# Toytiny/CMFlow

Hardware: AMD Instinct MI355X
Metric: frame-pairs/sec CMFlow fwd+bwd (higher is better)
Workload: dtype f32; 1 GPU; cmflow fwd+bwd training (7 cross-modal losses + Adam, train-mode BN) step, N=256, B=64 per GPU (global 64), ball-query r=2/4/8/16 K=4/8/16/32, kNN K=8; synthetic clouds, seeded random-init weights; parallelism=dp1

## Files before the change

### cmflow_amd/_lib.py

```python
import ctypes
import os
import subprocess

import torch

_HERE = os.path.dirname(os.path.abspath(__file__))
SO_PATH = os.environ.get("CMF_LIB") or os.path.join(_HERE, "libcmflow_hip.so")

_vp, _ci, _cf, _ll = ctypes.c_void_p, ctypes.c_int, ctypes.c_float, ctypes.c_longlong

SIGNATURES = {
    "cmf_ball_query": [_ci, _ci, _ci, _cf, _ci, _vp, _vp, _vp, _vp],
    "cmf_ball_query_multi": [_ci, _ci, _ci, _ci, _vp, _vp, _ci, _vp, _vp, _vp, _ci, _vp],
    "cmf_setconv_queries": [_ci, _vp, _vp],
    "cmf_ball_query_multi_counted": [_ci, _ci, _ci, _ci, _vp, _vp, _ci, _vp, _vp, _vp, _vp, _vp, _vp],
    "cmf_setconv_queries_counted": [_ci, _vp, _vp, _vp],
    "cmf_knn_counted": [_ci, _ci, _ci, _ci, _vp, _vp, _vp, _vp, _vp, _vp],
    "cmf_global_max_cat_counted": [_ci, _ci, _ci, _vp, _ll, _vp, _ll, _vp, _vp, _vp],
    "cmf_ego_refine_counted": [_ci, _ci, _cf, _cf, _vp, _vp, _vp, _vp, _vp, _vp, _vp, _vp, _vp, _vp, _vp, _vp],
    "cmf_eval_metrics_counted": [_ci, _ci, _vp, _vp, _vp, _vp, _vp, _vp, _vp, _vp, _cf, _cf, _cf, _vp, _vp, _vp],
    "cmf_ego_refine_grad_counted": [_ci, _ci, _cf, _vp, _vp, _vp, _vp, _vp, _vp, _vp, _vp, _vp, _vp, _vp, _vp, _vp],
    "cmf_global_max_cat_grad_counted": [_ci, _ci, _ci, _vp, _ll, _vp, _vp, _ll, _vp, _vp],
    "cmf_radar_loss_counted_workspace": [_ci, _ci, _ci, _ci],
    "cmf_radar_loss_counted_workspace_tiled": [_ci, _ci, _ci, _ci],
# ... 49 lines not shown
    "cmf_three_nn": [_ci, _ci, _ci, _vp, _vp, _vp, _vp, _vp],
    "cmf_three_interpolate": [_ci, _ci, _ci, _ci, _vp, _vp, _vp, _vp, _vp],
    "cmf_three_interpolate_grad": [_ci, _ci, _ci, _ci, _vp, _vp, _vp, _vp, _vp],
    "cmf_bn_finalize": [_ci, _ci, ctypes.c_double, _vp, _vp, _vp, _cf, _cf, _vp, _vp, _vp, _vp, _vp, _vp, _vp, _vp],
    "cmf_colsum_finalize": [_ci, _ci, _vp, _vp, _vp, _vp, _vp],
    "cmf_group_affine": [_ci, _ci, _ci, _ci, _ci, _vp, _ci, _vp, _ci, _vp, _vp, _vp, _ci, _vp, _ci, _vp, _vp, _vp, _vp, _vp],
    "cmf_adam_step": [_ci, _vp, _vp, _ll, _vp, _vp, _vp, ctypes.c_double, ctypes.c_double, ctypes.c_double, ctypes.c_double, ctypes.c_double, _ll, _vp],
    "cmf_group_prep": [_ci, _ci, _ci, _ci, _ci, _vp, _vp, _vp, _ci, _vp, _vp, _vp, _vp, _vp],
    "cmf_gemm_gather_affine": [_ci, _ci, _ci, _vp, _ll, _vp, _vp, _vp, _vp, _vp, _vp, _ll, _vp, _ll, _vp, _vp],
    "cmf_gemm_dx_gather": [_ci, _ci, _ci, _vp, _ll, _vp, _ll, _vp, _ll, _vp, _ll, _vp, _vp, _vp, _vp, _vp, _vp, _vp, _vp, _vp],
    "cmf_group_perm": [_ci, _ci, _vp, _vp, _vp, _vp, _vp, _vp, _vp],
    "cmf_gemm_dx_gather_sum": [_ci, _ci, _ci, _vp, _ll, _vp, _ll, _vp, _ll, _vp, _vp, _vp, _vp, _vp, _vp, _vp, _vp, _vp, _vp, _vp],
    "cmf_group_rows_grad_bn_cf_pieces": [_ci, _ci, _ci, _ci, _ci, _vp, _vp, _ll, _vp, _ll, _vp, _vp, _vp, _vp, _vp, _vp, _cf, _vp, _vp, _vp,
                                         _ci, _vp],
    "cmf_gemm_dw_gather_split": [_ci, _ci, _ll],
    "cmf_gemm_dw_gather_bn_bwd": [_ci, _ci, _ll, _vp, _ll, _vp, _ll, _vp, _vp, _vp, _vp, _vp, _ll, _vp, _ll, _vp, _vp, _vp, _vp, _vp, _vp, _ll,
                                  _ci, _vp, _ci, _vp],
    "cmf_gemm_dw_gather": [_ci, _ci, _ll, _vp, _ll, _vp, _ll, _vp, _vp, _vp, _vp, _vp, _vp, _ll, _ci, _vp, _ci, _vp],
    "cmf_colsum": [_ci, _ci, _vp, _vp, _ci, _vp, _vp, _vp],
    "cmf_setconv_dwx": [_ci, _cf, _ci, _vp, _vp, _vp, _vp, _vp, _vp, _ci, _ci, _vp],
    "cmf_group_rows_grad_bn": [_ci, _ci, _ci, _ci, _vp, _vp, _vp, _vp, _vp, _vp, _cf, _vp, _vp, _vp, _ci, _vp],
    "cmf_group_rows_grad_bn_cf": [_ci, _ci, _ci, _ci, _ci, _vp, _vp, _ll, _vp, _ll, _vp, _vp, _vp, _vp, _vp, _vp, _cf, _vp, _vp, _vp,
                                  _ci, _vp],
    "cmf_bn_relu_maxpool": [_ll, _ci, _ci, _vp, _vp, _vp, _vp, _ll, _vp, _vp],
    "cmf_maxpool_bwd": [_ll, _ci, _ci, _vp, _ll, _vp, _vp, _vp, _vp, _vp, _vp, _vp, _vp, _vp],
    "cmf_affine_relu": [_ll, _ci, _vp, _ll, _vp, _vp, _vp, _ll, _vp],
    "cmf_act_bwd_stats": [_ll, _ci, _vp, _ll, _vp, _ll, _vp, _vp, _vp, _vp, _vp, _vp, _vp],
    "cmf_bn_bwd_apply": [_ll, _ci, _vp, _vp, _ll, _vp, _vp, _vp, _vp, _vp],
    "cmf_maxpool_bwd_point": [_ll, _ci, _ci, _vp, _ll, _vp, _vp, _vp, _vp, _vp, _vp, _vp, _vp, _vp],
    "cmf_thin_bwd_layer_pooled": [_ll, _ci, _ci, _ci, _vp, _vp, _vp, _vp, _vp, _vp, _vp, _vp, _vp, _vp, _vp, _vp, _vp, _vp, _vp, _vp,
                                  _ci, _vp, _vp],
    "cmf_thin_bwd_wide_supported": [_ci, _ci],
    "cmf_thin_bwd_wide_slabs": [_ll, _ci, _vp],
    "cmf_thin_bwd_wide_layer": [_ll, _ci, _vp, _ll, _vp, _vp, _ci, _vp, _ll, _vp, _vp, _vp, _vp, _vp, _ll, _vp, _ll,
                                _vp, _vp, _vp, _vp, _vp, _ll, _vp, _vp, _ll, _ci, _vp, _vp],
    "cmf_thin_bwd_supported": [_ci, _ci],
    "cmf_thin_bwd_slabs": [_ll, _vp],
    "cmf_thin_bwd_layer": [_ll, _ci, _ci, _vp, _ll, _vp, _ll, _vp, _vp, _vp, _vp, _vp, _ll, _vp, _ll, _ci,
                           _vp, _vp, _vp, _vp, _vp, _vp, _ll, _vp, _vp, _ll, _ci, _vp, _vp],
    "cmf_weighted_ksum": [_ll, _ci, _ci, _ci, _ci, _vp, _vp, _vp, _vp, _vp],
    "cmf_weighted_ksum_grad_tiles": [_ci],
    "cmf_weighted_ksum_grad": [_ll, _ci, _ci, _ci, _ci, _ci, _vp, _vp, _vp, _vp, _vp, _vp, _vp, _vp],
    "cmf_weightnet_ksum_tiles": [_ci],
    "cmf_weightnet_ksum": [_ll, _ci, _ci, _ci, _ci, _vp, _vp, _vp, _vp, _vp, _vp, _vp],
    "cmf_weightnet_ksum_grad": [_ll, _ci, _ci, _ci, _ci, _ci, _vp, _ll, _vp, _vp, _vp, _vp, _vp, _vp, _vp, _vp, _vp],
    "cmf_global_max_cat": [_ci, _ci, _ci, _vp, _ll, _vp, _ll, _vp, _vp],
# ... 168 lines not shown
```

### cmflow_amd/csrc/cmf_common.h

```cpp
#pragma once
#include <hip/hip_runtime.h>
#include <atomic>
#include <mutex>
#include <stdint.h>
#include <stdlib.h>

#define CMF_WAVE 64

#define CMF_CHECK_ARG(cond) \
    do { if (!(cond)) return (int)hipErrorInvalidValue; } while (0)

static inline int cmf_launch_status() { return (int)hipGetLastError(); }

static inline int cmf_divup(long long a, long long b) { return (int)((a + b - 1) / b); }

static inline bool cmf_env_on(const char *name)
{
    const char *e = getenv(name);
    return !(e && e[0] == '0');
}

struct CmfPerDevice {
    std::atomic<unsigned> mask[4] = {};
    bool need(int &dev) { dev = 0; (void)hipGetDevice(&dev); return dev >= 128 || !(mask[dev >> 5].load(std::memory_order_acquire) & (1u << (dev & 31))); }
// ... 33 lines not shown
struct CmfGroupAffineArgs { int b, n_src, P, S, C; const float *ysrc; int ld_src; const float *xyz_src, *xyz_ctr, *Wx; int ldw; const int *idx;
                            float *z, *dxyz, *partial, *partial_x; };
struct CmfPoolArgs { long long P; int S, C; const float *z, *a, *c; float *out; long long ldo; unsigned char *argmax; int grid; float *zsel; };
struct CmfPoolBwdArgs { long long P; int S, C; const float *dout; long long ldd; const float *z, *a, *c, *mean, *invstd; const unsigned char *argmax;
                        float *g, *partial; int sel; };
struct CmfInverseArgs { int n, P, S; const int *idx; int *offsets, *inv; };
struct CmfDwxArgs { int C; float inv_count; int train; const float *bwd5, *fwd, *a, *mean, *invstd; float *dwx; int ld, accumulate; };
struct CmfScatterArgs { int n, entries, S; const float *dU, *y; long long ldy; const float *wx; long long ldw; const float *xyz_src, *xyz_ctr,
                        *a, *mean, *invstd, *sums; float inv_count; const int *offsets, *inv; float *grad_feat; int ldg; };
struct CmfChainInferArgs { long long M; int N, S; const int *idx; const float *xyz, *y; long long ldy; const float *wx; long long ldwx;
                           const float *bn0, *bn1, *bn2, *w2, *w3; float *out; long long ldo; };
int cmf_setconv_chain_infer_batch(int n, const CmfChainInferArgs *q, void *stream);
struct CmfSplitkArgs { int M, N, split_k; const float *workspace; float *C; long long ldc; int accumulate; };
struct CmfThinBwdCall { long long rows; int cout, cin; const float *dU; long long lddu; const float *z; long long ldz;
                        const float *a, *mean, *invstd, *sums; const float *w; long long ldw; const float *x; long long ldx; int in_mode;
                        const float *a_in, *c_in, *mean_in, *invstd_in; float *dx; long long lddx; float *stats;
                        float *dw; long long lddw; int accumulate; float *slabs; int nslab;
                        const float *dxyz; const float *pool_g; const unsigned char *pool_am; int pool_S; };
int cmf_bn_finalize_batch(int n, const CmfBnFinArgs *a, hipStream_t st);
int cmf_colsum_batch(int n, const CmfColsumArgs *a, hipStream_t st);
int cmf_maxpool_bwd_point_batch(int n, const CmfPoolBwdArgs *a, hipStream_t st);
int cmf_setconv_dwx_batch(int n, const CmfDwxArgs *a, hipStream_t st);
int cmf_build_inverse_ps_batch(int n, int b, const CmfInverseArgs *a, hipStream_t st);
int cmf_group_rows_grad_bn_cf_batch(int n, int b, int c, const CmfScatterArgs *a, hipStream_t st);
int cmf_group_affine_batch(int n, const CmfGroupAffineArgs *a, hipStream_t st);
int cmf_bn_relu_maxpool_batch(int n, CmfPoolArgs *a, hipStream_t st);
int cmf_act_bwd_stats_batch(int n, const CmfActBwdArgs *a, hipStream_t st);
int cmf_affine_relu_batch(int n, const CmfAffineArgs *a, hipStream_t st);
int cmf_splitk_reduce_batch(int n, const CmfSplitkArgs *a, hipStream_t st);
int cmf_thin_fwd_batch(int n, const GemmArgs *g, hipStream_t st);
int cmf_thin_bwd_layer_batch(int n, CmfThinBwdCall *c, hipStream_t st);

bool cmf_setconv_chain_supported(int N, int S, int O1, int C2, int C3, long long M);
long long cmf_setconv_chain_waves(long long M, int backward);
int cmf_setconv_chain_pass(int mode, long long M, int N, int S, const int *idx, const float *xyz, const float *y, long long ldy, const float *wx,
                           long long ldwx, const float *bn0, const float *bn1, const float *bn2, const float *w2, const float *w3, float *out,
                           long long ldo, float *zsel, unsigned char *argmax, float *partial, const float *g, const float *dU_in, float *dU_out,
                           float *slabs, void *stream);
int cmf_setconv_chain_infer(long long M, int N, int S, const int *idx, const float *xyz, const float *y, long long ldy, const float *wx,
                            long long ldwx, const float *bn0, const float *bn1, const float *bn2, const float *w2, const float *w3, float *out,
                            long long ldo, void *stream);
int cmf_bn_relu_maxpool_sel(long long P, int S, int C, const float *z, const float *a, const float *c, float *out, long long ldo,
                            unsigned char *argmax, float *zsel, void *stream);
int cmf_maxpool_bwd_point_sel(long long P, int C, const float *dout, long long ldd, const float *zsel, const float *a, const float *c,
                              const float *mean, const float *invstd, float *g, float *partial, void *stream);
int cmf_colsum_store(int tiles, int ncols, const float *partial, float *out, int C, float *dst0, float *dst1, void *stream);
// ... 3 lines not shown
```

### cmflow_amd/csrc/group_rows.hip

```cpp
#include <algorithm>
#include "cmf_common.h"
#include "../../include/cmflow_hip.h"

int cmf_build_inverse_rows(int b, int n, int P, int S, const int *idx, int *offsets, int *inv, void *stream, int entries);

constexpr int GR_THREADS = 256;

template <int VEC>
__global__ __launch_bounds__(GR_THREADS) void group_rows_kernel(
    int n, int c, int ldf, int entries, long long total_vec,
    const float *__restrict__ feat, const int *__restrict__ idx, float *__restrict__ out)
{
    const int cv = c / VEC;
    for (long long i = (long long)blockIdx.x * GR_THREADS + threadIdx.x; i < total_vec;
         i += (long long)gridDim.x * GR_THREADS) {
        const long long row = i / cv;
        const int col = (int)(i - row * cv) * VEC;
        const int bs = (int)(row / entries);
        const int j = idx[row];
        const float *src = feat + ((size_t)bs * n + j) * ldf + col;
        float *dst = out + (size_t)row * c + col;
        if (VEC == 4) *reinterpret_cast<float4 *>(dst) = *reinterpret_cast<const float4 *>(src);
        else *dst = *src;
    }
// ... 188 lines not shown
    }
    if (t == 0) off[n] = base;
    __threadfence_block();
    __syncthreads();
    if (t < P)
        for (int s = 0; s < S; ++s) {
            const int j = ix[t * S + s];
            lst[off[j] + cnt[t * ld + j] + rk[t * S + s]] = t * S + s;
        }
}

__global__ __launch_bounds__(INVM_THREADS) void inverse_matrix_kernel(
    int n, int P, int S, const int *__restrict__ idx, int *__restrict__ offsets, int *__restrict__ inv)
{
    inverse_matrix_body(n, P, S, idx, offsets, inv);
}

__global__ __launch_bounds__(INVM_THREADS) void inverse_matrix_batch_kernel(const CmfBatch<CmfInverseArgs> b)
{
    const CmfInverseArgs &p = b.a[blockIdx.y];
    inverse_matrix_body(p.n, p.P, p.S, p.idx, p.offsets, p.inv);
}

int cmf_build_inverse_ps_batch(int n, int b, const CmfInverseArgs *a, hipStream_t st)
{
    CMF_CHECK_ARG(n >= 1 && n <= CMF_MAX_BATCH && a && b > 0);
    CmfBatch<CmfInverseArgs> bt;
    size_t mat = 0;
    for (int i = 0; i < n; ++i) {
        const CmfInverseArgs &q = a[i];
        const size_t m = (((size_t)q.P * (q.n | 1) + 7) / 8) * 16 + (size_t)q.P * q.S;
        CMF_CHECK_ARG(q.n > 0 && q.n < 40000 && q.P > 0 && q.P <= INVM_THREADS && q.S > 0 && q.S <= 64 && m <= 150 * 1024 && q.idx && q.offsets && q.inv);
        bt.a[i] = q;
        mat = std::max(mat, m);
    }
    static CmfPerDevice attr_set;
    int attr_dev;
    if (attr_set.need(attr_dev)) {
        (void)hipFuncSetAttribute((const void *)inverse_matrix_batch_kernel, hipFuncAttributeMaxDynamicSharedMemorySize, 150 * 1024);
        attr_set.done(attr_dev);
    }
    hipLaunchKernelGGL(inverse_matrix_batch_kernel, dim3(b, n), dim3(INVM_THREADS), mat, st, bt);
    return cmf_launch_status();
}

extern "C" int cmf_build_inverse(int b, int n, int entries, const int *idx, int *offsets, int *inv, void *stream)
{
    CMF_CHECK_ARG(b >= 0 && n > 0 && entries >= 0 && n < 40000);
    if (b == 0) return 0;
    CMF_CHECK_ARG(idx && offsets && inv);
    return cmf_build_inverse_rows(b, n, 0, 0, idx, offsets, inv, stream, entries);
}

extern "C" int cmf_build_inverse_ps(int b, int n, int P, int S, const int *idx, int *offsets, int *inv, void *stream)
{
// ... 223 lines not shown
        for (; t < end; ++t) {
            const float4 u0 = *(const float4 *)(gu + (size_t)lst[t] * c + col);
            acc.x += u0.x; acc.y += u0.y; acc.z += u0.z; acc.w += u0.w;
        }
        const float4 sa = *(const float4 *)(a + col);
        float r[4] = {acc.x, acc.y, acc.z, acc.w};
        if (sums) {
            const float4 t1 = *(const float4 *)(sums + col), t2 = *(const float4 *)(sums + c + col);
            const float4 is = *(const float4 *)(invstd + col), mu = *(const float4 *)(mean + col);
            const float4 yv = *(const float4 *)(y + ((size_t)bs * n + j) * ldy + col);
            const float s1[4] = {t1.x, t1.y, t1.z, t1.w}, s2[4] = {t2.x, t2.y, t2.z, t2.w}, iv[4] = {is.x, is.y, is.z, is.w};
            const float ym[4] = {yv.x - mu.x, yv.y - mu.y, yv.z - mu.z, yv.w - mu.w};
#pragma unroll
            for (int i = 0; i < 4; ++i) {
                const float *w = wx + (size_t)(col + i) * ldw;
                const float zsum = cnt * ym[i] + (w[0] * Dx + w[1] * Dy + w[2] * Dz);
                r[i] = r[i] - cnt * (s1[i] * inv_count) - (iv[i] * s2[i] * inv_count) * zsum;
            }
        }
        *(float4 *)(dst + col) = make_float4(sa.x * r[0], sa.y * r[1], sa.z * r[2], sa.w * r[3]);
    }
}

template <int LPP>
__device__ __forceinline__ void group_rows_grad_bn_cf_narrow_body(
    int n, int entries, int S, long long points, const float *__restrict__ dU, const float *__restrict__ y, long long ldy,
    const float *__restrict__ wx, long long ldw, const float *__restrict__ xyz_src, const float *__restrict__ xyz_ctr,
    const float *__restrict__ a, const float *__restrict__ mean, const float *__restrict__ invstd,
    const float *__restrict__ sums, float inv_count,
    const int *__restrict__ offsets, const int *__restrict__ inv, float *__restrict__ grad_feat, int ldg)
{
    constexpr int PPW = CMF_WAVE / LPP, c = LPP * 4;
    const long long gwave = ((long long)blockIdx.x * GR_THREADS + threadIdx.x) / CMF_WAVE;
    const int lane = threadIdx.x % CMF_WAVE, sub = lane / LPP, sl = lane % LPP;
    const long long pt = gwave * PPW + sub;
    const bool live = pt < points;
    const int bs = live ? (int)(pt / n) : 0, j = live ? (int)(pt - (long long)bs * n) : 0;
    const int *off = offsets + (size_t)bs * (n + 1);
    const int beg = live ? off[j] : 0, end = live ? off[j + 1] : 0;
    const int *lst = inv + (size_t)bs * entries;
    const float *gu = dU + (size_t)bs * entries * c;
    const int col = sl * 4;
    float Dx = 0.f, Dy = 0.f, Dz = 0.f;
    constexpr bool MERGED = LPP == 8;
    const float *xs = xyz_src + ((size_t)bs * n + j) * 3;
    const float *xc = xyz_ctr + (size_t)bs * (entries / S) * 3;
// ... 169 lines not shown
```

### cmflow_amd/csrc/setconv_block.hip

```cpp
#include <algorithm>
#include <condition_variable>
#include <cstdint>
#include <functional>
#include <mutex>
#include <thread>
#include <vector>
#include "cmf_common.h"
#include "gemm_args.h"
#include "../../include/cmflow_hip.h"

namespace {

#define CMF_TRY(call) do { int e_ = (call); if (e_) return e_; } while (0)

inline bool thin_fused_on() { static const bool on = cmf_env_on("CMF_THIN_FUSED"); return on; }
inline bool thin_wide_on() { static const bool on = cmf_env_on("CMF_THIN_WIDE"); return on; }
inline bool body_batch_on() { static const bool on = cmf_env_on("CMF_BODY_BATCH"); return on; }
inline bool tail_batch_on() { static const bool on = cmf_env_on("CMF_TAIL_BATCH"); return on; }
inline bool train_gather_on() { static const bool on = cmf_env_on("CMF_TRAIN_GATHER"); return on; }
inline bool train_gather_sum_on() { static const bool on = cmf_env_on("CMF_TRAIN_GATHER_SUM"); return on; }
inline bool bnb_gather_on() { static const bool on = cmf_env_on("CMF_BNB_GATHER"); return on; }

inline int setconv_path(const cmf_setconv_desc *d)
{
// ... 55 lines not shown
    float *dxyz, *z1, *z2, *z3, *x, *z4, *z5, *z6, *fwd_sums;
    unsigned char *argmax;
    float *zsel;
    Bn bn[6];
    float *partial, *partial_x, *sums, *t6, *t5, *t4, *dx, *dU3, *dU2, *dU1, *splitk;
    float *dZ2;
    size_t saved_floats, scratch_floats;
    float *z(int l) const { float *const v[6] = {z1, z2, z3, z4, z5, z6}; return v[l]; }
    float *dU(int l) const { float *const v[6] = {dU1, dU2, dU3, t4, t5, t6}; return v[l]; }
    float *zin(int l) const { return l == 3 ? x : z(l - 1); }
    float *dUin(int l) const { return l == 3 ? dx : dU(l - 1); }
    Bn bn_in(int l) const { return l == 3 ? Bn() : bn[l - 1]; }
};

inline int chan(const cmf_setconv_desc *d, int layer)
{
    return layer == 0 ? d->O1 : d->C[layer - 1];
}
inline long long rows_of(const cmf_setconv_desc *d, int layer)
{
    return (long long)d->B * d->N * (layer <= 2 ? d->S : 1);
}

inline bool gather_layout(const cmf_setconv_desc *d)
{
    const long long M = (long long)d->B * d->N * d->S;
    return train_gather_on() && M % 128 == 0 && M < (1ll << 31) && d->C[0] % 128 == 0 && d->O1 % 128 == 0 && d->ldy % 4 == 0;
}
inline bool gather_sum_shape(const cmf_setconv_desc *d) { return train_gather_sum_on() && gather_layout(d) && d->S >= 2; }
inline bool gather_sum_layout(const cmf_setconv_desc *d) { return gather_sum_shape(d) && d->dy != nullptr; }

inline bool bnb_gather(const cmf_setconv_desc *d)
{
    return bnb_gather_on() && d->training && gather_layout(d) && ((long long)d->B * d->N * d->S) >= 32768;
}

Layout make_layout(const cmf_setconv_desc *d, float *saved, float *scratch, bool backward, bool sum_in_gemm = false)
{
    Layout L;
    const long long P = (long long)d->B * d->N, M = P * d->S;
    const int O1 = d->O1, C2 = d->C[0], C3 = d->C[1], C4 = d->C[2], C5 = d->C[3], C6 = d->C[4];
    Bump s(saved);
    L.idx = (int *)s.take(M);
    L.offsets = (int *)s.take((size_t)d->B * (d->N + 1));
    L.inv = (int *)s.take(M);
    L.dxyz = s.take(M * 4);
    L.z1 = s.take(gather_layout(d) ? (size_t)((M + 3) / 4 * 4) + 3 * (size_t)O1 : (size_t)M * O1);
    L.z2 = s.take(M * C2);
    L.z3 = s.take(M * C3);
    L.argmax = (unsigned char *)s.take((P * C3 + 3) / 4);
    L.x = s.take(P * C3);
// ... 249 lines not shown
    float *const slabs = split > 1 ? L.splitk : nullptr;
    CMF_TRY(bn_grad_sums(bn_grad_args(d, L, 1, tiles128(M)), st));
    const float *dZ2 = L.dU2;
    if (bnb_gather(d) && L.dZ2 && d->dw[0]) {
        CMF_TRY(cmf_gemm_dw_gather_bn_bwd(C2, O1, M, L.dU2, C2, L.z2, C2, b.a, b.mean, b.invstd, L.sums, L.dZ2, C2, d->y, d->ldy, rows, L.dxyz, wx3,
                                          b0.a, b0.c, d->dw[0], O1, split, slabs, d->acc_w[0], st));
        dZ2 = L.dZ2;
    } else {
        CMF_TRY(cmf_bn_bwd_apply(M, C2, L.dU2, L.z2, C2, b.a, b.mean, b.invstd, d->training ? L.sums : nullptr, st));
        if (d->dw[0])
            CMF_TRY(cmf_gemm_dw_gather(C2, O1, M, L.dU2, C2, d->y, d->ldy, rows, L.dxyz, wx3, b0.a, b0.c, d->dw[0], O1, split, slabs, d->acc_w[0], st));
    }
    if (gather_sum_layout(d)) {
        const SumSlots q = sum_slots(d, L);
        CMF_TRY(cmf_group_perm(d->B, d->N * d->S, L.inv, rows, L.dxyz, q.perm, q.pts, q.dq2, st));
        cmf_gemm_dx_gather_sum_hint((long long)d->B * d->N);
        return cmf_gemm_dx_gather_sum((int)M, O1, C2, dZ2, C2, d->w[0], O1, d->y, d->ldy, q.perm, q.pts, q.dq2, wx3, b0.a, b0.c, b0.mean, b0.invstd,
                                      q.pieces, L.partial, st);
    }
    return cmf_gemm_dx_gather((int)M, O1, C2, dZ2, C2, d->w[0], O1, L.dU1, O1, d->y, d->ldy, rows, L.dxyz, wx3, b0.a, b0.c, b0.mean, b0.invstd,
                              L.partial, st);
}

}

extern "C" int cmf_setconv_sizes(const cmf_setconv_desc *d, long long *saved_floats, long long *scratch_fwd, long long *scratch_bwd,
                                 long long *scratch_bwd_input_grad)
{
    CMF_CHECK_ARG(d && d->B > 0 && d->N > 0 && d->S > 0 && d->S <= 64 && d->O1 % 4 == 0);
    for (int i = 0; i < 5; ++i) CMF_CHECK_ARG(d->C[i] > 0 && d->C[i] % 4 == 0);
    const Layout f = make_layout(d, nullptr, nullptr, false);
    if (saved_floats) *saved_floats = (long long)f.saved_floats;
    if (scratch_fwd) *scratch_fwd = (long long)f.scratch_floats;
    if (scratch_bwd) *scratch_bwd = (long long)make_layout(d, nullptr, nullptr, true, false).scratch_floats;
    if (scratch_bwd_input_grad) *scratch_bwd_input_grad = (long long)make_layout(d, nullptr, nullptr, true, true).scratch_floats;
    return 0;
}

static int setconv_forward_part(const cmf_setconv_desc *d, void *st, int part)
{
    CMF_CHECK_ARG(d && d->xyz && d->y && d->wx && d->saved && d->scratch && d->out);
    CMF_CHECK_ARG(!gather_layout(d) || gather_operands_aligned(d));
    const Layout L = make_layout(d, d->saved, d->scratch, false);
    const long long P = (long long)d->B * d->N, M = P * d->S;
    const int O1 = d->O1, C2 = d->C[0], C3 = d->C[1];
    const Bn &b0 = L.bn[0], &b2 = L.bn[2];
    if (!d->training) CMF_TRY(fold_all_eval(d, L, st));
    if (!d->idx_ready) CMF_TRY(cmf_ball_query_defined(d->B, d->N, d->N, d->radius, d->S, d->xyz, d->xyz, L.idx, st));
    if (setconv_path(d) == 1) {
        CMF_TRY(cmf_setconv_chain_infer(M, d->N, d->S, L.idx, d->xyz, d->y, d->ldy, d->wx, d->ldwx, L.bn[0].block(), L.bn[1].block(),
                                        L.bn[2].block(), d->w[0], d->w[1], L.x, C3, st));
    } else if (chain_train(d)) {
        CMF_TRY(cmf_setconv_chain_pass(1, M, d->N, d->S, L.idx, d->xyz, d->y, d->ldy, d->wx, d->ldwx, L.bn[0].block(), L.bn[1].block(),
                                       L.bn[2].block(), d->w[0], d->w[1], L.x, C3, L.z3, L.argmax, L.partial, nullptr, nullptr, nullptr, nullptr, st));
    } else {
        const bool gather = gather_layout(d) || (!d->training && d->inference && M % 128 == 0 && C2 % 128 == 0 && O1 % 16 == 0 &&
                                                 d->ldy % 4 == 0 && gather_operands_aligned(d) && M < (1ll << 31));
        if (gather) {
            if (d->training) {
                CMF_TRY(cmf_group_affine(d->B, d->N, d->N, d->S, O1, d->y, (int)d->ldy, nullptr, 0, d->xyz, d->xyz, d->wx, (int)d->ldwx, L.idx, 0,
                                         nullptr, L.dxyz, L.partial, L.partial_x, st));
                CMF_TRY(cmf_colsum(tiles128(M), 3 * O1 + 4, L.partial_x, L.fwd_sums, 0, nullptr, nullptr, st));
                CMF_TRY(fold(d, L, 0, st));
            }
            CMF_TRY(cmf_group_prep(d->B, d->N, d->N, d->S, O1, d->xyz, d->xyz, d->wx, (int)d->ldwx, L.idx, gather_rows(L), L.dxyz,
                                   gather_wx3(L, M), st));
            CMF_TRY(cmf_gemm_gather_affine((int)M, C2, O1, d->y, d->ldy, gather_rows(L), L.dxyz, gather_wx3(L, M), b0.a, b0.c, d->w[0], O1,
                                           L.z2, C2, d->training ? L.partial : nullptr, st));
        } else {
            CMF_TRY(cmf_group_affine(d->B, d->N, d->N, d->S, O1, d->y, (int)d->ldy, nullptr, 0, d->xyz, d->xyz, d->wx, (int)d->ldwx, L.idx, 0,
                                     L.z1, L.dxyz, d->training ? L.partial : nullptr, d->training ? L.partial_x : nullptr, st));
            if (d->training) CMF_TRY(cmf_colsum(tiles128(M), 3 * O1 + 4, L.partial_x, L.fwd_sums, 0, nullptr, nullptr, st));
            CMF_TRY(fold(d, L, 0, st));
            CMF_TRY(fwd_gemm(fwd_layer(d, L, 1), st));
        }
        CMF_TRY(fold(d, L, 1, st));
        CMF_TRY(fwd_gemm(fwd_layer(d, L, 2), st));
        CMF_TRY(fold(d, L, 2, st));
        CMF_TRY(cmf_bn_relu_maxpool_sel(P, d->S, C3, L.z3, b2.a, b2.c, L.x, C3, L.argmax, L.zsel, st));
    }
    return part == 1 ? 0 : forward_tail(d, L, st);
}

extern "C" int cmf_setconv_forward(const cmf_setconv_desc *d, void *st) { return setconv_forward_part(d, st, 0); }

extern "C" int cmf_setconv_path(const cmf_setconv_desc *d) { return d ? setconv_path(d) : 0; }

static int setconv_queries(int n, const cmf_setconv_desc *descs, const int *const *counts, void *stream)
{
    CMF_CHECK_ARG(n >= 0 && (n == 0 || descs));
    int i = 0;
    while (i < n) {
        const cmf_setconv_desc &d0 = descs[i];
        CMF_CHECK_ARG(d0.xyz && d0.saved);
        int nq = 1;
        while (i + nq < n && nq < 4 && descs[i + nq].xyz == d0.xyz && descs[i + nq].B == d0.B && descs[i + nq].N == d0.N) ++nq;
// ... 20 lines not shown
            }
        } else {
            float radii[4];
            int ns[4];
            const float *ctr[2], *cloud[2];
            int *idx[8];
            for (int c = 0; c < nclouds; ++c) {
                ctr[c] = cloud[c] = descs[i + c * nq].xyz;
                for (int q = 0; q < nq; ++q) {
                    const cmf_setconv_desc &d = descs[i + c * nq + q];
                    CMF_CHECK_ARG(d.saved);
                    idx[c * nq + q] = make_layout(&d, d.saved, nullptr, false).idx;
                    if (c == 0) { radii[q] = d.radius; ns[q] = d.S; }
                }
            }
            if (counts) {
                const int *cnt[2] = {counts[i], counts[i + (nclouds - 1) * nq]};
                CMF_TRY(cmf_ball_query_multi_counted(d0.B, d0.N, d0.N, nq, radii, ns, nclouds, ctr, cloud, idx, cnt, cnt, stream));
            } else
                CMF_TRY(cmf_ball_query_multi(d0.B, d0.N, d0.N, nq, radii, ns, nclouds, ctr, cloud, idx, 1, stream));
        }
        i += nq * nclouds;
    }
    return 0;
}

extern "C" int cmf_setconv_queries(int n, const cmf_setconv_desc *descs, void *stream) { return setconv_queries(n, descs, nullptr, stream); }

extern "C" int cmf_setconv_queries_counted(int n, const cmf_setconv_desc *descs, const int *const *counts, void *stream)
{
    CMF_CHECK_ARG(n == 0 || counts);
    return setconv_queries(n, descs, counts, stream);
}

static bool tail_batchable(int n, const cmf_setconv_desc *descs)
{
    if (!tail_batch_on() || n < 1 || n > CMF_MAX_BATCH) return false;
    for (int i = 0; i < n; ++i) {
        const cmf_setconv_desc &d = descs[i];
        for (int k = 1; k < 5; ++k)
            if (d.C[k] > 64 || d.C[k] % 32 || d.C[k] != descs[0].C[k]) return false;
        if (d.training != descs[0].training || ((long long)d.B * d.N) % 128) return false;
        for (int k = 2; k < 5; ++k) if (!d.dw[k] && descs[0].dw[k]) return false;
    }
    return true;
}

// ... 46 lines not shown
        CmfSplitkArgs sk[CMF_MAX_BATCH];
        for (int i = 0; i < n; ++i) {
            tb[i] = bwd_layer_args(&descs[i], L[i], l);
            cs[i] = bn_grad_args(&descs[i], L[i], l, tiles128(tb[i].rows));
        }
        CMF_TRY(cmf_colsum_batch(n, cs, st));
        CMF_TRY(cmf_thin_bwd_layer_batch(n, tb, st));
        for (int i = 0; i < n; ++i) sk[i] = splitk_args(tb[i]);
        CMF_TRY(cmf_splitk_reduce_batch(n, sk, st));
    }
    return 0;
}

static int setconv_backward_part(const cmf_setconv_desc *d, void *st, int part)
{
    CMF_CHECK_ARG(d && d->xyz && d->saved && d->scratch && d->dout);
    CMF_CHECK_ARG(!gather_layout(d) || (d->y && gather_operands_aligned(d)));
    const Layout L = make_layout(d, d->saved, d->scratch, true, d->dy != nullptr);
    const long long P = (long long)d->B * d->N, M = P * d->S;
    const int O1 = d->O1, C2 = d->C[0], C3 = d->C[1];
    const Bn &b0 = L.bn[0];
    const bool chain = chain_train(d);
    const int wv = chain ? (int)cmf_setconv_chain_waves(M, 1) : 0;
    if (d->dy) CMF_TRY(cmf_build_inverse_ps(d->B, d->N, d->N, d->S, L.idx, L.offsets, L.inv, st));
    if (part != 2) CMF_TRY(backward_tail(d, L, st));
    float *g = L.dU3;
    const CmfThinBwdCall q = bwd_layer_args(d, L, 2);
    const bool fused = thin_fused_on() && M % 128 == 0 && d->dw[1];
    if (chain) {
        const float *bn0 = L.bn[0].block(), *bn1 = L.bn[1].block(), *bn2 = L.bn[2].block();
        const int nslab = wv / 4;
        CMF_TRY(pooled_grad_head(d, L, L.z3, st));
        CMF_TRY(cmf_setconv_chain_pass(2, M, d->N, d->S, L.idx, d->xyz, d->y, d->ldy, d->wx, d->ldwx, bn0, bn1, bn2, d->w[0], d->w[1],
                                       nullptr, 0, nullptr, L.argmax, L.partial, g, nullptr, L.dU2, L.splitk, st));
        if (d->dw[1]) CMF_TRY(cmf_splitk_reduce(C3, C2, nslab, L.splitk, d->dw[1], C2, d->acc_w[1], (hipStream_t)st));
        CMF_TRY(bn_grad_sums(bn_grad_args(d, L, 1, wv), st));
        CMF_TRY(cmf_setconv_chain_pass(3, M, d->N, d->S, L.idx, d->xyz, d->y, d->ldy, d->wx, d->ldwx, bn0, bn1, bn2, d->w[0], d->w[1],
                                       nullptr, 0, nullptr, nullptr, L.partial, nullptr, L.dU2, L.dU1, L.splitk, st));
        if (d->dw[0]) CMF_TRY(cmf_splitk_reduce(C2, O1, nslab, L.splitk, d->dw[0], O1, d->acc_w[0], (hipStream_t)st));
    } else {
        if (fused && cmf_thin_bwd_supported(C3, C2) && C3 % 32 == 0 && C2 % 32 == 0) {
            CMF_TRY(pooled_grad_head(d, L, L.zsel, st));
            CMF_TRY(cmf_thin_bwd_layer_pooled(P, d->S, q.cout, q.cin, g, L.argmax, q.z, q.a, q.mean, q.invstd, q.sums, q.w, q.x, q.a_in, q.c_in,
                                              q.mean_in, q.invstd_in, q.dx, q.stats, q.dw, q.accumulate, q.slabs, st));
        } else if (fused && thin_wide_on() && cmf_thin_bwd_wide_supported(C3, C2)) {
            CMF_TRY(pooled_grad_head(d, L, L.zsel, st));
            CMF_TRY(cmf_thin_bwd_wide_layer(q.rows, q.cin, nullptr, q.lddu, g, L.argmax, d->S, q.z, q.ldz, q.a, q.mean, q.invstd, q.sums, q.w, q.ldw,
// ... 463 lines not shown
```

### include/cmflow_hip.h

```cpp
#ifndef CMFLOW_HIP_H
#define CMFLOW_HIP_H

#ifdef __cplusplus
extern "C" {
#endif


int cmf_ball_query(int b, int n, int m, float radius, int nsample,
                   const float *new_xyz, const float *xyz, int *idx, void *stream);
int cmf_ball_query_multi(int b, int n, int m, int nq, const float *radii, const int *nsamples, int nclouds,
                         const float *const *new_xyz, const float *const *xyz, int *const *idx, int zero_empty, void *stream);

int cmf_group_points(int b, int c, int n, int npoints, int nsample,
                     const float *points, const int *idx, float *out, void *stream);

int cmf_group_points_grad(int b, int c, int n, int npoints, int nsample,
                          const float *grad_out, const int *idx, float *grad_points, void *stream);

int cmf_query_and_group(int b, int n, int m, float radius, int nsample, int c, int use_xyz,
                        const float *new_xyz, const float *xyz, const float *features, int *idx, float *out, void *stream);


int cmf_knn(int b, int n, int s, int nsample, const float *xyz, const float *new_xyz,
            int *idx, float *dist, void *stream);
// ... 124 lines not shown
                              void *stream);

int cmf_thin_bwd_wide_supported(int cout, int cin);
int cmf_thin_bwd_wide_slabs(long long rows, int cin, int *tiles_per_workgroup);
int cmf_thin_bwd_wide_layer(long long rows, int cin, const float *dU, long long lddu, const float *pool_g,
                            const unsigned char *pool_am, int pool_S, const float *z, long long ldz,
                            const float *a, const float *mean, const float *invstd, const float *sums,
                            const float *w, long long ldw, const float *x, long long ldx,
                            const float *a_in, const float *c_in, const float *mean_in, const float *invstd_in,
                            float *dx, long long lddx, float *stats, float *dw, long long lddw, int accumulate, float *slabs,
                            void *stream);

int cmf_group_rows_grad_bn(int b, int n, int c, int entries, const float *dU, const float *z,
                           const float *a, const float *mean, const float *invstd, const float *sums,
                           float inv_count, const int *offsets, const int *inv, float *grad_feat, int ldg, void *stream);
int cmf_group_rows_grad_bn_cf(int b, int n, int c, int entries, int S, const float *dU, const float *y, long long ldy,
                              const float *wx, long long ldw, const float *xyz_src, const float *xyz_ctr,
                              const float *a, const float *mean, const float *invstd, const float *sums,
                              float inv_count, const int *offsets, const int *inv, float *grad_feat, int ldg, void *stream);
int cmf_group_rows_grad_bn_cf_pieces(int b, int n, int c, int entries, int S, const float *pieces, const float *y, long long ldy,
                                     const float *wx, long long ldw, const float *xyz_src, const float *xyz_ctr,
                                     const float *a, const float *mean, const float *invstd, const float *sums,
                                     float inv_count, const int *offsets, const int *inv, float *grad_feat, int ldg, void *stream);

int cmf_setconv_dwx(int C, float inv_count, int train, const float *bwd5, const float *fwd,
                    const float *a, const float *mean, const float *invstd, float *dwx, int ld, int accumulate,
                    void *stream);

int cmf_gather_points(int b, int c, int n, int npoints, const float *points, const int *idx, float *out, void *stream);
int cmf_gather_points_grad(int b, int c, int n, int npoints, const float *grad_out, const int *idx,
                           float *grad_points, void *stream);
int cmf_furthest_point_sampling(int b, int n, int m, const float *dataset, float *temp, int *idxs, void *stream);
int cmf_knn_points(int b, int n, int m, int k, const float *unknown, const float *known,
                   float *dist2, int *idx, void *stream);
int cmf_three_nn(int b, int n, int m, const float *unknown, const float *known, float *dist2, int *idx, void *stream);
int cmf_three_interpolate(int b, int c, int m, int n, const float *points, const int *idx,
                          const float *weight, float *out, void *stream);
int cmf_three_interpolate_grad(int b, int c, int n, int m, const float *grad_out, const int *idx,
                               const float *weight, float *grad_points, void *stream);

typedef struct cmf_setconv_desc {
    int B, N, S;
    int O1;
    int C[5];
    float radius;
    int training;
// ... 166 lines not shown
```

Baseline: 3414 frame-pairs/s.

## Compute first-layer BN stats per source point via inverse index lists

```diff
diff --git a/cmflow_amd/_lib.py b/cmflow_amd/_lib.py
--- a/cmflow_amd/_lib.py
+++ b/cmflow_amd/_lib.py
@@ -95,6 +95,7 @@
     "cmf_group_rows_grad_bn": [_ci, _ci, _ci, _ci, _vp, _vp, _vp, _vp, _vp, _vp, _cf, _vp, _vp, _vp, _ci, _vp],
     "cmf_group_rows_grad_bn_cf": [_ci, _ci, _ci, _ci, _ci, _vp, _vp, _ll, _vp, _ll, _vp, _vp, _vp, _vp, _vp, _vp, _cf, _vp, _vp, _vp,
                                   _ci, _vp],
+    "cmf_group_stats_cf": [_ci, _ci, _ci, _ci, _ci, _vp, _ll, _vp, _vp, _vp, _ll, _vp, _vp, _vp, _vp, _vp],
     "cmf_bn_relu_maxpool": [_ll, _ci, _ci, _vp, _vp, _vp, _vp, _ll, _vp, _vp],
     "cmf_maxpool_bwd": [_ll, _ci, _ci, _vp, _ll, _vp, _vp, _vp, _vp, _vp, _vp, _vp, _vp, _vp],
     "cmf_affine_relu": [_ll, _ci, _vp, _ll, _vp, _vp, _vp, _ll, _vp],
diff --git a/cmflow_amd/csrc/cmf_common.h b/cmflow_amd/csrc/cmf_common.h
--- a/cmflow_amd/csrc/cmf_common.h
+++ b/cmflow_amd/csrc/cmf_common.h
@@ -79,6 +79,7 @@
 int cmf_maxpool_bwd_point_batch(int n, const CmfPoolBwdArgs *a, hipStream_t st);
 int cmf_setconv_dwx_batch(int n, const CmfDwxArgs *a, hipStream_t st);
 int cmf_build_inverse_ps_batch(int n, int b, const CmfInverseArgs *a, hipStream_t st);
+bool cmf_inverse_matrix_takes(int n, int P, int S);
 int cmf_group_rows_grad_bn_cf_batch(int n, int b, int c, const CmfScatterArgs *a, hipStream_t st);
 int cmf_group_affine_batch(int n, const CmfGroupAffineArgs *a, hipStream_t st);
 int cmf_bn_relu_maxpool_batch(int n, CmfPoolArgs *a, hipStream_t st);
diff --git a/cmflow_amd/csrc/group_rows.hip b/cmflow_amd/csrc/group_rows.hip
--- a/cmflow_amd/csrc/group_rows.hip
+++ b/cmflow_amd/csrc/group_rows.hip
@@ -234,6 +234,12 @@
     inverse_matrix_body(p.n, p.P, p.S, p.idx, p.offsets, p.inv);
 }
 
+static inline size_t invm_lds(int n, int P, int S) { return (((size_t)P * (n | 1) + 7) / 8) * 16 + (size_t)P * S; }
+bool cmf_inverse_matrix_takes(int n, int P, int S)
+{
+    return n > 0 && n < 40000 && P > 0 && P <= INVM_THREADS && S > 0 && S <= 64 && invm_lds(n, P, S) <= 150 * 1024;
+}
+
 int cmf_build_inverse_ps_batch(int n, int b, const CmfInverseArgs *a, hipStream_t st)
 {
     CMF_CHECK_ARG(n >= 1 && n <= CMF_MAX_BATCH && a && b > 0);
@@ -241,8 +247,8 @@
     size_t mat = 0;
     for (int i = 0; i < n; ++i) {
         const CmfInverseArgs &q = a[i];
-        const size_t m = (((size_t)q.P * (q.n | 1) + 7) / 8) * 16 + (size_t)q.P * q.S;
-        CMF_CHECK_ARG(q.n > 0 && q.n < 40000 && q.P > 0 && q.P <= INVM_THREADS && q.S > 0 && q.S <= 64 && m <= 150 * 1024 && q.idx && q.offsets && q.inv);
+        const size_t m = invm_lds(q.n, q.P, q.S);
+        CMF_CHECK_ARG(cmf_inverse_matrix_takes(q.n, q.P, q.S) && q.idx && q.offsets && q.inv);
         bt.a[i] = q;
         mat = std::max(mat, m);
     }
@@ -512,6 +518,130 @@
     }
 }
 
+constexpr int GS_THREADS = 1024, GS_WAVES = GS_THREADS / CMF_WAVE, GS_POINTS = 128, GS_PPW = GS_POINTS / GS_WAVES, GS_COLS = CMF_WAVE * 4;
+
+__device__ __forceinline__ double gs_wave_sum(double v)
+{
+#pragma unroll
+    for (int m = CMF_WAVE / 2; m > 0; m >>= 1) v += __shfl_xor(v, m, CMF_WAVE);
+    return v;
+}
+
+__device__ __forceinline__ void gs_reduce_store(const double (&v)[4], double (*red)[GS_COLS], float *__restrict__ out, int cols)
+{
+    const int lane = threadIdx.x % CMF_WAVE, wave = threadIdx.x / CMF_WAVE;
+    __syncthreads();
+#pragma unroll
+    for (int i = 0; i < 4; ++i) red[wave][lane * 4 + i] = v[i];
+    __syncthreads();
+    if ((int)threadIdx.x < cols) {
+        double s = 0.0;
+#pragma unroll
+        for (int w = 0; w < GS_WAVES; ++w) s += red[w][threadIdx.x];
+        out[threadIdx.x] = (float)s;
+    }
+}
+
+__global__ __launch_bounds__(GS_THREADS) void group_stats_cf_kernel(
+    int n, int C, int entries, int S, int points, const float *__restrict__ y, long long ldy, int y_vec,
+    const float *__restrict__ wx, long long ldw, const float *__restrict__ xyz_src, const float *__restrict__ xyz_ctr,
+    const int *__restrict__ offsets, const int *__restrict__ inv, float *__restrict__ partial, float *__restrict__ partial_x)
+{
+    __shared__ double red[GS_WAVES][GS_COLS];
+    __shared__ double red_u[GS_WAVES][3];
+    const int lane = threadIdx.x % CMF_WAVE, wave = threadIdx.x / CMF_WAVE;
+    const int col0 = blockIdx.y * GS_COLS, col = col0 + lane * 4;
+    const bool live = col < C;
+    const int ctrs = entries / S;
+    float w[4][3];
+#pragma unroll
+    for (int i = 0; i < 4; ++i)
+#pragma unroll
+        for (int k = 0; k < 3; ++k) w[i][k] = live ? wx[(size_t)(col + i) * ldw + k] : 0.f;
+    double s1[4] = {0.0, 0.0, 0.0, 0.0}, s2[4] = {0.0, 0.0, 0.0, 0.0};
+    double tz[3][4] = {{0.0, 0.0, 0.0, 0.0}, {0.0, 0.0, 0.0, 0.0}, {0.0, 0.0, 0.0, 0.0}};
+    double u[3] = {0.0, 0.0, 0.0};
+    const int pt0 = blockIdx.x * GS_POINTS + wave * GS_PPW;
+    int lbeg = 0, lend = 0;
+    if (lane < GS_PPW && pt0 + lane < points) {
+        const int bs = (pt0 + lane) / n, j = (pt0 + lane) - bs * n;
+        const int *off = offsets + (size_t)bs * (n + 1);
+        lbeg = off[j]; lend = off[j + 1];
+    }
+    for (int k = 0; k < GS_PPW; ++k) {
+        const int pt = pt0 + k;
+        const int beg = __shfl(lbeg, k, CMF_WAVE), end = __shfl(lend, k, CMF_WAVE);
+        if (pt >= points || end <= beg) continue;
+        const int bs = pt / n;
+        float yv[4] = {0.f, 0.f, 0.f, 0.f};
+        if (live) {
+            const float *yp = y + (size_t)pt * ldy + col;
+            if (y_vec) { const float4 v = *(const float4 *)yp; yv[0] = v.x; yv[1] = v.y; yv[2] = v.z; yv[3] = v.w; }
+            else { yv[0] = yp[0]; yv[1] = yp[1]; yv[2] = yp[2]; yv[3] = yp[3]; }
+        }
+        const float *xs = xyz_src + (size_t)pt * 3;
+        const float sx = xs[0], sy = xs[1], sz = xs[2];
+        const float *xc = xyz_ctr + (size_t)bs * ctrs * 3;
+        const int *lst = inv + (size_t)bs * entries;
+        double D[3] = {0.0, 0.0, 0.0}, E[6] = {0.0, 0.0, 0.0, 0.0, 0.0, 0.0};
+        for (int t = beg + lane; t < end; t += CMF_WAVE) {
+            const int p = lst[t] / S;
+            const double dx = (double)(sx - xc[p * 3]), dy = (double)(sy - xc[p * 3 + 1]), dz = (double)(sz - xc[p * 3 + 2]);
+            D[0] += dx; D[1] += dy; D[2] += dz;
+            E[0] += dx * dx; E[1] += dx * dy; E[2] += dx * dz; E[3] += dy * dy; E[4] += dy * dz; E[5] += dz * dz;
+        }
+#pragma unroll
+        for (int q = 0; q < 3; ++q) D[q] = gs_wave_sum(D[q]);
+#pragma unroll
+        for (int q = 0; q < 6; ++q) E[q] = gs_wave_sum(E[q]);
+        const double cnt = (double)(end - beg);
+        u[0] += D[0]; u[1] += D[1]; u[2] += D[2];
+#pragma unroll
+        for (int i = 0; i < 4; ++i) {
+            const double yy = (double)yv[i], w0 = (double)w[i][0], w1 = (double)w[i][1], w2 = (double)w[i][2];
+            const double a = w0 * D[0] + w1 * D[1] + w2 * D[2];
+            const double e0 = E[0] * w0 + E[1] * w1 + E[2] * w2;
+            const double e1 = E[1] * w0 + E[3] * w1 + E[4] * w2;
+            const double e2 = E[2] * w0 + E[4] * w1 + E[5] * w2;
+            s1[i] += cnt * yy + a;
+            s2[i] += cnt * yy * yy + 2.0 * yy * a + (w0 * e0 + w1 * e1 + w2 * e2);
+            tz[0][i] += yy * D[0] + e0; tz[1][i] += yy * D[1] + e1; tz[2][i] += yy * D[2] + e2;
+        }
+    }
+    const int cols = min(GS_COLS, C - col0);
+    float *pr = partial + (size_t)blockIdx.x * 2 * C + col0;
+    float *px = partial_x + (size_t)blockIdx.x * (3 * C + 4) + col0;
+    gs_reduce_store(s1, red, pr, cols);
+    gs_reduce_store(s2, red, pr + C, cols);
+    gs_reduce_store(tz[0], red, px, cols);
+    gs_reduce_store(tz[1], red, px + C, cols);
+    gs_reduce_store(tz[2], red, px + 2 * C, cols);
+    if (blockIdx.y == 0) {
+        if (lane == 0) { red_u[wave][0] = u[0]; red_u[wave][1] = u[1]; red_u[wave][2] = u[2]; }
+        __syncthreads();
+        if (threadIdx.x < 4) {
+            double s = 0.0;
+            if (threadIdx.x < 3)
+                for (int q = 0; q < GS_WAVES; ++q) s += red_u[q][threadIdx.x];
+            partial_x[(size_t)blockIdx.x * (3 * C + 4) + 3 * C + threadIdx.x] = (float)s;
+        }
+    }
+}
+
+extern "C" int cmf_group_stats_cf(int b, int n_src, int P, int S, int C, const float *y, long long ldy, const float *xyz_src, const float *xyz_ctr,
+                                  const float *wx, long long ldw, const int *offsets, const int *inv, float *partial, float *partial_x, void *stream)
+{
+    CMF_CHECK_ARG(b >= 0 && n_src > 0 && P > 0 && S > 0 && C > 0 && C % 4 == 0 && ldy >= C && ldw >= 3);
+    CMF_CHECK_ARG((long long)b * n_src < (1ll << 31) && (long long)P * S < (1ll << 31));
+    if (b == 0) return 0;
+    CMF_CHECK_ARG(y && xyz_src && xyz_ctr && wx && offsets && inv && partial && partial_x);
+    const int points = b * n_src;
+    const int y_vec = (ldy % 4 == 0 && ((uintptr_t)y & 15) == 0) ? 1 : 0;
+    hipLaunchKernelGGL(group_stats_cf_kernel, dim3(cmf_divup(points, GS_POINTS), cmf_divup(C, GS_COLS)), dim3(GS_THREADS), 0, (hipStream_t)stream,
+                       n_src, C, P * S, S, points, y, ldy, y_vec, wx, ldw, xyz_src, xyz_ctr, offsets, inv, partial, partial_x);
+    return cmf_launch_status();
+}
+
 template <int LPP>
 __device__ __forceinline__ void group_rows_grad_bn_cf_narrow_body(
     int n, int entries, int S, long long points, const float *__restrict__ dU, const float *__restrict__ y, long long ldy,
diff --git a/cmflow_amd/csrc/setconv_block.hip b/cmflow_amd/csrc/setconv_block.hip
--- a/cmflow_amd/csrc/setconv_block.hip
+++ b/cmflow_amd/csrc/setconv_block.hip
@@ -101,11 +101,13 @@
     return (long long)d->B * d->N * (layer <= 2 ? d->S : 1);
 }
 
-inline bool gather_layout(const cmf_setconv_desc *d)
+inline bool gather_shape(const cmf_setconv_desc *d)
 {
     const long long M = (long long)d->B * d->N * d->S;
-    return train_gather_on() && M % 128 == 0 && M < (1ll << 31) && d->C[0] % 128 == 0 && d->O1 % 128 == 0 && d->ldy % 4 == 0;
-}
+    return M % 128 == 0 && M < (1ll << 31) && d->C[0] % 128 == 0 && d->O1 % 128 == 0 && d->ldy % 4 == 0;
+}
+inline bool gather_layout(const cmf_setconv_desc *d) { return train_gather_on() && gather_shape(d); }
+inline bool stats_cf(const cmf_setconv_desc *d) { return d->training && gather_shape(d); }
 inline bool gather_sum_shape(const cmf_setconv_desc *d) { return train_gather_sum_on() && gather_layout(d) && d->S >= 2; }
 inline bool gather_sum_layout(const cmf_setconv_desc *d) { return gather_sum_shape(d) && d->dy != nullptr; }
 
@@ -401,6 +403,33 @@
                               L.partial, st);
 }
 
+int first_layer_stats_cf(const cmf_setconv_desc *d, const Layout &L, void *st)
+{
+    const int O1 = d->O1, rows = tiles128((long long)d->B * d->N);
+    CMF_TRY(cmf_group_stats_cf(d->B, d->N, d->N, d->S, O1, d->y, d->ldy, d->xyz, d->xyz, d->wx, d->ldwx, L.offsets, L.inv, L.partial,
+                               L.partial_x, st));
+    CMF_TRY(cmf_colsum(rows, 3 * O1 + 4, L.partial_x, L.fwd_sums, 0, nullptr, nullptr, st));
+    CmfBnFinArgs f = fold_args(d, L, 0);
+    f.tiles = rows;
+    return bn_finalize(f, st);
+}
+
+int build_inverses_fwd(int n, const cmf_setconv_desc *descs, void *st)
+{
+    CmfInverseArgs iv[CMF_MAX_BATCH];
+    int nb = 0, B = 0;
+    for (int i = 0; i < n; ++i) {
+        const cmf_setconv_desc &d = descs[i];
+        if (!stats_cf(&d) || d.B <= 0) continue;
+        const Layout L = make_layout(&d, d.saved, nullptr, false);
+        if (!cmf_inverse_matrix_takes(d.N, d.N, d.S)) { CMF_TRY(cmf_build_inverse_ps(d.B, d.N, d.N, d.S, L.idx, L.offsets, L.inv, st)); continue; }
+        if (nb == CMF_MAX_BATCH || (nb > 0 && d.B != B)) { CMF_TRY(cmf_build_inverse_ps_batch(nb, B, iv, (hipStream_t)st)); nb = 0; }
+        B = d.B;
+        iv[nb++] = CmfInverseArgs{d.N, d.N, d.S, L.idx, L.offsets, L.inv};
+    }
+    return nb ? cmf_build_inverse_ps_batch(nb, B, iv, (hipStream_t)st) : 0;
+}
+
 }
 
 extern "C" int cmf_setconv_sizes(const cmf_setconv_desc *d, long long *saved_floats, long long *scratch_fwd, long long *scratch_bwd,
@@ -425,7 +454,10 @@
     const int O1 = d->O1, C2 = d->C[0], C3 = d->C[1];
     const Bn &b0 = L.bn[0], &b2 = L.bn[2];
     if (!d->training) CMF_TRY(fold_all_eval(d, L, st));
-    if (!d->idx_ready) CMF_TRY(cmf_ball_query_defined(d->B, d->N, d->N, d->radius, d->S, d->xyz, d->xyz, L.idx, st));
+    if (!d->idx_ready) {
+        CMF_TRY(cmf_ball_query_defined(d->B, d->N, d->N, d->radius, d->S, d->xyz, d->xyz, L.idx, st));
+        CMF_TRY(build_inverses_fwd(1, d, st));
+    }
     if (setconv_path(d) == 1) {
         CMF_TRY(cmf_setconv_chain_infer(M, d->N, d->S, L.idx, d->xyz, d->y, d->ldy, d->wx, d->ldwx, L.bn[0].block(), L.bn[1].block(),
                                         L.bn[2].block(), d->w[0], d->w[1], L.x, C3, st));
@@ -435,22 +467,21 @@
     } else {
         const bool gather = gather_layout(d) || (!d->training && d->inference && M % 128 == 0 && C2 % 128 == 0 && O1 % 16 == 0 &&
                                                  d->ldy % 4 == 0 && gather_operands_aligned(d) && M < (1ll << 31));
+        const bool cf = stats_cf(d);
         if (gather) {
-            if (d->training) {
-                CMF_TRY(cmf_group_affine(d->B, d->N, d->N, d->S, O1, d->y, (int)d->ldy, nullptr, 0, d->xyz, d->xyz, d->wx, (int)d->ldwx, L.idx, 0,
-                                         nullptr, L.dxyz, L.partial, L.partial_x, st));
-                CMF_TRY(cmf_colsum(tiles128(M), 3 * O1 + 4, L.partial_x, L.fwd_sums, 0, nullptr, nullptr, st));
-                CMF_TRY(fold(d, L, 0, st));
-            }
+            if (d->training) CMF_TRY(first_layer_stats_cf(d, L, st));
             CMF_TRY(cmf_group_prep(d->B, d->N, d->N, d->S, O1, d->xyz, d->xyz, d->wx, (int)d->ldwx, L.idx, gather_rows(L), L.dxyz,
                                    gather_wx3(L, M), st));
             CMF_TRY(cmf_gemm_gather_affine((int)M, C2, O1, d->y, d->ldy, gather_rows(L), L.dxyz, gather_wx3(L, M), b0.a, b0.c, d->w[0], O1,
                                            L.z2, C2, d->training ? L.partial : nullptr, st));
         } else {
             CMF_TRY(cmf_group_affine(d->B, d->N, d->N, d->S, O1, d->y, (int)d->ldy, nullptr, 0, d->xyz, d->xyz, d->wx, (int)d->ldwx, L.idx, 0,
-                                     L.z1, L.dxyz, d->training ? L.partial : nullptr, d->training ? L.partial_x : nullptr, st));
-            if (d->training) CMF_TRY(cmf_colsum(tiles128(M), 3 * O1 + 4, L.partial_x, L.fwd_sums, 0, nullptr, nullptr, st));
-            CMF_TRY(fold(d, L, 0, st));
+                                     L.z1, L.dxyz, d->training && !cf ? L.partial : nullptr, d->training && !cf ? L.partial_x : nullptr, st));
+            if (cf) CMF_TRY(first_layer_stats_cf(d, L, st));
+            else {
+                if (d->training) CMF_TRY(cmf_colsum(tiles128(M), 3 * O1 + 4, L.partial_x, L.fwd_sums, 0, nullptr, nullptr, st));
+                CMF_TRY(fold(d, L, 0, st));
+            }
             CMF_TRY(fwd_gemm(fwd_layer(d, L, 1), st));
         }
         CMF_TRY(fold(d, L, 1, st));
@@ -517,7 +548,7 @@
         }
         i += nq * nclouds;
     }
-    return 0;
+    return build_inverses_fwd(n, descs, stream);
 }
 
 extern "C" int cmf_setconv_queries(int n, const cmf_setconv_desc *descs, void *stream) { return setconv_queries(n, descs, nullptr, stream); }
@@ -610,7 +641,7 @@
     const Bn &b0 = L.bn[0];
     const bool chain = chain_train(d);
     const int wv = chain ? (int)cmf_setconv_chain_waves(M, 1) : 0;
-    if (d->dy) CMF_TRY(cmf_build_inverse_ps(d->B, d->N, d->N, d->S, L.idx, L.offsets, L.inv, st));
+    if (d->dy && !stats_cf(d)) CMF_TRY(cmf_build_inverse_ps(d->B, d->N, d->N, d->S, L.idx, L.offsets, L.inv, st));
     if (part != 2) CMF_TRY(backward_tail(d, L, st));
     float *g = L.dU3;
     const CmfThinBwdCall q = bwd_layer_args(d, L, 2);
diff --git a/include/cmflow_hip.h b/include/cmflow_hip.h
--- a/include/cmflow_hip.h
+++ b/include/cmflow_hip.h
@@ -170,6 +170,9 @@
                                      const float *wx, long long ldw, const float *xyz_src, const float *xyz_ctr,
                                      const float *a, const float *mean, const float *invstd, const float *sums,
                                      float inv_count, const int *offsets, const int *inv, float *grad_feat, int ldg, void *stream);
+
+int cmf_group_stats_cf(int b, int n_src, int P, int S, int C, const float *y, long long ldy, const float *xyz_src, const float *xyz_ctr,
+                       const float *wx, long long ldw, const int *offsets, const int *inv, float *partial, float *partial_x, void *stream);
 
 int cmf_setconv_dwx(int C, float inv_count, int train, const float *bwd5, const float *fwd,
                     const float *a, const float *mean, const float *invstd, float *dwx, int ld, int accumulate,
```

Result: no change. 3406 frame-pairs/s (-0.2%).
